# roysubhankar/dwt-domain-adaptation

Measured on NVIDIA H100. Metric: ResNet-50-DWT images/sec fwd+bwd, higher is better.
Workload: dtype f32

## Files before the change

dwt-domain-adaptation_b200/dwt_b200/csrc/norm_cl.cu:

```cuda
#include <stdlib.h>

#include <type_traits>

#include <cuda_bf16.h>

#include "dwt_common.cuh"
#include "norm_launch.h"
#include "small_algebra.cuh"

namespace dwt {
namespace {

constexpr int kT = 256;

__device__ __forceinline__ void pdl_wait() { asm volatile("griddepcontrol.wait;" ::: "memory"); }
__device__ __forceinline__ void pdl_launch_dependents() { asm volatile("griddepcontrol.launch_dependents;" ::: "memory"); }

template <int GS> struct ClShape {
  static constexpr int NSUB = 4 / GS;
  static constexpr int NM = GS * (GS + 1) / 2;
  static constexpr int FWD1 = GS + NM;
  static constexpr int BWD1 = GS * GS + GS;
  static constexpr int FWD = NSUB * FWD1;
  static constexpr int BWD = NSUB * BWD1;
};

struct ClThread {
  int C4, CW, LS, rpi, col, rsub, q;
  bool active;
  __device__ __forceinline__ ClThread(const Geom& gm) {
    C4 = gm.C >> 2;
    CW = gm.cw;
    LS = gm.ls;
    rpi = kT / LS;
    col = threadIdx.x % LS;
    rsub = threadIdx.x / LS;
    q = blockIdx.y * CW + col;
    active = col < CW && rsub < rpi && q < C4;
  }
};

template <int UNROLL, bool DESC, class F>
__device__ __forceinline__ void sweep_rows(const ClThread& t, unsigned rows, F&& body) {
  const unsigned krows = (unsigned)t.rpi * UNROLL, nch = (rows + krows - 1) / krows;
  for (unsigned i = blockIdx.x; i < nch; i += gridDim.x) body((DESC ? nch - 1 - i : i) * krows + t.rsub);
}
#define CL_FOR_DOMAINS(d, gm, DESC) \
  for (int di_ = blockIdx.z, d = (DESC) ? (gm).D - 1 - di_ : di_; di_ < (gm).D; di_ += gridDim.z, d = (DESC) ? (gm).D - 1 - di_ : di_)

template <class T> constexpr bool kBf16 = !std::is_same<T, float>::value;
template <class T>
__device__ __forceinline__ float as_stored(float v) {
  if constexpr (kBf16<T>) return __bfloat162float(__float2bfloat16_rn(v));
  else return v;
}

template <int NACC>
__device__ __forceinline__ void column_reduce(const ClThread& t, float (&acc)[NACC], float* sRed) {
  if (t.rpi == 1) return;
  if (t.rsub < t.rpi) {
#pragma unroll
    for (int i = 0; i < NACC; ++i) sRed[i * kT + threadIdx.x] = acc[i];
  }
  __syncthreads();
  if (t.rsub == 0) {
#pragma unroll
    for (int i = 0; i < NACC; ++i) {
      float s = acc[i];
      for (int r = 1; r < t.rpi; ++r) s += sRed[i * kT + r * t.LS + t.col];
      acc[i] = s;
    }
  }
}

template <class T, int GS>
__global__ void __launch_bounds__(kT, 3) cl_stats_kernel(const T* __restrict__ x, const Geom gm,
                                                         float* __restrict__ partial, float* __restrict__ shift) {
  using S = ClShape<GS>;
  constexpr int UNROLL = 8;
  __shared__ float sRed[kT * S::FWD];
  const ClThread t(gm);
  const unsigned rows = (unsigned)gm.N * gm.HW;
  pdl_launch_dependents();
  CL_FOR_DOMAINS(d, gm, true) {
    const T* xd = x + (size_t)d * rows * gm.C + 4 * t.q;
    float K[4] = {0.f, 0.f, 0.f, 0.f};
    if (t.active) {
      const unsigned np = rows < 8 ? rows : 8;
      for (unsigned r = 0; r < np; ++r) {
        const float4 v = ld4(xd + (size_t)r * gm.C);
        K[0] += v.x; K[1] += v.y; K[2] += v.z; K[3] += v.w;
      }
#pragma unroll
      for (int c = 0; c < 4; ++c) K[c] /= (float)np;
      if (rows > 8) {
        float s1[4] = {0.f, 0.f, 0.f, 0.f}, s2[4] = {0.f, 0.f, 0.f, 0.f};
        const size_t mid = (size_t)gm.HW / 2 + (size_t)sqrtf((float)gm.HW) / 2;
        for (unsigned k = 0; k < 8; ++k) {
          const float4 v = ld4(xd + ((2 * (size_t)k + 1) * rows / 16 + mid) % rows * gm.C);
          const float e[4] = {v.x - K[0], v.y - K[1], v.z - K[2], v.w - K[3]};
#pragma unroll
          for (int c = 0; c < 4; ++c) { s1[c] += e[c]; s2[c] = fmaf(e[c], e[c], s2[c]); }
        }
#pragma unroll
        for (int c = 0; c < 4; ++c) {
          const float dk = s1[c] * 0.125f;
          if (401.f * dk * dk > 400.f * (s2[c] * 0.125f)) K[c] += dk;
        }
      }
      if (blockIdx.x == 0 && t.rsub == 0) *reinterpret_cast<float4*>(shift + (size_t)d * gm.C + 4 * t.q) = make_float4(K[0], K[1], K[2], K[3]);
    }
    float acc[S::FWD];
#pragma unroll
    for (int i = 0; i < S::FWD; ++i) acc[i] = 0.f;
    if (t.active) sweep_rows<UNROLL, true>(t, rows, [&](unsigned r) {
      float4 v[UNROLL];
#pragma unroll
      for (int u = 0; u < UNROLL; ++u) {
        const unsigned rr = r + u * t.rpi;
        v[u] = rr < rows ? ld4(xd + (size_t)rr * gm.C) : make_float4(K[0], K[1], K[2], K[3]);
      }
#pragma unroll
      for (int u = 0; u < UNROLL; ++u) {
        const float e[4] = {v[u].x - K[0], v[u].y - K[1], v[u].z - K[2], v[u].w - K[3]};
#pragma unroll
        for (int s = 0; s < S::NSUB; ++s) {
#pragma unroll
          for (int c = 0; c < GS; ++c) {
            acc[s * S::FWD1 + c] += e[s * GS + c];
#pragma unroll
            for (int j = 0; j <= c; ++j)
              acc[s * S::FWD1 + GS + c * (c + 1) / 2 + j] = fmaf(e[s * GS + c], e[s * GS + j], acc[s * S::FWD1 + GS + c * (c + 1) / 2 + j]);
          }
        }
      }
    });
    column_reduce<S::FWD>(t, acc, sRed);
    if (t.rsub == 0 && t.active) {
      float* dst = partial + (((size_t)d * gridDim.x + blockIdx.x) * t.C4 + t.q) * S::FWD;
#pragma unroll
      for (int i = 0; i < S::FWD; ++i) dst[i] = acc[i];
    }
    if (gridDim.z == 1) __syncthreads();
  }
}

template <int GS, int PER>
__device__ __forceinline__ int acc_index(int g, int a) {
  constexpr int NSUB = 4 / GS;
  return (g / NSUB) * (NSUB * PER) + (g % NSUB) * PER + a;
}

constexpr int kFinQ = 2;

template <int NACC>
__device__ __forceinline__ void column_row_sum(const float* __restrict__ col, int nrows, int W, float (&a)[NACC]) {
  static_assert(NACC % 2 == 0, "accumulators are read as float2");
#pragma unroll
  for (int i = 0; i < NACC; ++i) a[i] = 0.f;
#pragma unroll 4
  for (int r = threadIdx.x; r < nrows; r += 32) {
    const float2* p = reinterpret_cast<const float2*>(col + (size_t)r * W);
#pragma unroll
    for (int i = 0; i < NACC / 2; ++i) {
      const float2 v = __ldcg(p + i);
      a[2 * i] += v.x; a[2 * i + 1] += v.y;
    }
  }
#pragma unroll
  for (int o = 1; o < 32; o <<= 1)
#pragma unroll
    for (int i = 0; i < NACC; ++i) a[i] += __shfl_xor_sync(0xffffffffu, a[i], o);
}

template <int NSUB, int PER>
__device__ __forceinline__ void take_group(const float (&a)[NSUB * PER], int s, float (&v)[PER]) {
#pragma unroll
  for (int i = 0; i < PER; ++i) {
    v[i] = a[i];
#pragma unroll
    for (int k = 1; k < NSUB; ++k)
      if (s == k) v[i] = a[k * PER + i];
  }
}

template <int GS>
__device__ __forceinline__ void cl_fwd_finalize_site(const float* __restrict__ partial, int nrows, const float* __restrict__ shift,
                                                     const Geom& gm, const FwdFin& fin) {
  using SH = ClShape<GS>;
  constexpr int NST = GS + GS * GS;
  __shared__ float sStat[DWT_MAX_DOMAINS][kFinQ][SH::NSUB][NST + 1];
  __shared__ unsigned char sBad[DWT_MAX_DOMAINS][kFinQ][SH::NSUB];
  const int s = threadIdx.x, ql = threadIdx.y, d = threadIdx.z, q = blockIdx.x * blockDim.y + ql;
  const int W = (gm.C >> 2) * SH::FWD;
  const float invM = 1.f / gm.M;
  const bool colok = q < (gm.C >> 2);
  const bool lead = colok && s < SH::NSUB;
  const int g = q * SH::NSUB + (lead ? s : 0);
  const bool direct = gm.D == 1 || fin.aliased == 0;
  const int dbuf = direct ? d : 0;
  const bool upd = fin.update_running && lead && (direct || (fin.aliased == 1 && d == 0));
  float rc_old[GS * GS], rm_old[GS];
  if (upd) {
#pragma unroll
    for (int e = 0; e < GS * GS; ++e) rc_old[e] = fin.rcov[dbuf][(size_t)g * GS * GS + e];
#pragma unroll
    for (int e = 0; e < GS; ++e) rm_old[e] = fin.rmean[dbuf][g * GS + e];
  }
  pdl_launch_dependents();
  pdl_wait();
  float a[SH::FWD];
  if (colok) column_row_sum<SH::FWD>(partial + (size_t)d * nrows * W + (size_t)q * SH::FWD, nrows, W, a);
  if (lead) {
    float v[SH::FWD1];
    take_group<SH::NSUB, SH::FWD1>(a, s, v);
    float mean[GS], cov[GS][GS];
#pragma unroll
    for (int i = 0; i < GS; ++i) mean[i] = shift[(size_t)d * gm.C + g * GS + i] + v[i] * invM;
#pragma unroll
    for (int i = 0; i < GS; ++i)
#pragma unroll
      for (int j = 0; j <= i; ++j) {
        const float c = v[GS + i * (i + 1) / 2 + j] * invM - (v[i] * invM) * (v[j] * invM);
        cov[i][j] = c; cov[j][i] = c;
      }
    const bool bad = factor_thread<GS>(gm, fin, d, g, mean, cov, false);
    if (fin.update_running) {
      if (direct) {
        if (!bad) {
          const float m = fin.momentum, kk = 1.f - fin.momentum;
#pragma unroll
          for (int i = 0; i < GS; ++i) {
            fin.rmean[d][g * GS + i] = m * mean[i] + kk * rm_old[i];
#pragma unroll
            for (int j = 0; j < GS; ++j)
              fin.rcov[d][(size_t)g * GS * GS + i * GS + j] = m * (cov[i][j] * fin.unbias) + kk * rc_old[i * GS + j];
          }
        }
      } else {
        sBad[d][ql][s] = bad ? 1 : 0;
#pragma unroll
        for (int i = 0; i < GS; ++i) {
          sStat[d][ql][s][i] = mean[i];
#pragma unroll
          for (int j = 0; j < GS; ++j) sStat[d][ql][s][GS + i * GS + j] = cov[i][j];
        }
      }
    }
  }
  if (!fin.update_running || direct) return;
  __syncthreads();
  if (!(lead && d == 0)) return;
  if (fin.aliased == 1) {
    const float m = fin.momentum, kk = 1.f - fin.momentum;
    float* rc = fin.rcov[0] + (size_t)g * GS * GS;
    float* rm = fin.rmean[0] + g * GS;
    for (int dd = 0; dd < gm.D; ++dd) {
      if (sBad[dd][ql][s]) continue;
#pragma unroll
      for (int e = 0; e < GS * GS; ++e) rc_old[e] = m * (sStat[dd][ql][s][GS + e] * fin.unbias) + kk * rc_old[e];
#pragma unroll
      for (int e = 0; e < GS; ++e) rm_old[e] = m * sStat[dd][ql][s][e] + kk * rm_old[e];
    }
#pragma unroll
    for (int e = 0; e < GS * GS; ++e) rc[e] = rc_old[e];
#pragma unroll
    for (int e = 0; e < GS; ++e) rm[e] = rm_old[e];
  } else {
    for (int dd = 0; dd < gm.D; ++dd)
      if (!sBad[dd][ql][s]) ema_direct<GS>(gm, fin, dd, g, &sStat[dd][ql][s][0], &sStat[dd][ql][s][GS]);
  }
}

template <int GS>
__global__ void __launch_bounds__(32 * kFinQ * DWT_MAX_DOMAINS) cl_fwd_finalize_kernel(const float* __restrict__ partial, size_t pstride, int nrows,
                                                                                      const float* __restrict__ shift, size_t sstride, const Geom gm,
                                                                                      const __grid_constant__ FwdFin fin, const __grid_constant__ FwdFin fin2) {
  const bool second = blockIdx.y != 0;
  cl_fwd_finalize_site<GS>(partial + (second ? pstride : 0), nrows, shift + (second ? sstride : 0), gm, second ? fin2 : fin);
}

template <class T, int GS, int EPI, bool DS>
__global__ void __launch_bounds__(kT, 3) cl_apply_kernel(const T* __restrict__ x, T* __restrict__ y, const Geom gm,
                                                         const float* __restrict__ save_mean, const float* __restrict__ save_w,
                                                         const float* __restrict__ gamma, const float* __restrict__ beta,
                                                         const T* __restrict__ res, uint8_t* __restrict__ mask,
                                                         const float* __restrict__ save_mean_d, const float* __restrict__ save_w_d,
                                                         const float* __restrict__ gamma_d, const float* __restrict__ beta_d) {
  using S = ClShape<GS>;
  constexpr bool RES = (EPI & DWT_EPI_RESIDUAL) != 0;
  static_assert(!DS || RES, "the two-site tail is a residual epilogue");
  constexpr int UNROLL = DS ? 2 : (RES ? 4 : 8);
  const ClThread t(gm);
  if (!t.active) return;
  const unsigned rows = (unsigned)gm.N * gm.HW;
  pdl_wait();
  CL_FOR_DOMAINS(d, gm, false) {
    float Wp[S::NSUB][S::NM], bp[S::NSUB][GS], Wd[DS ? S::NSUB : 1][S::NM], bd[DS ? S::NSUB : 1][GS];
#pragma unroll
    for (int s = 0; s < S::NSUB; ++s) {
      const int g = t.q * S::NSUB + s;
      load_forward_map<GS, EPI>(save_w + ((size_t)d * gm.G + g) * GS * GS, save_mean + (size_t)d * gm.C + g * GS,
                                gamma + g * GS, beta + g * GS, Wp[s], bp[s]);
      if constexpr (DS)
        load_forward_map<GS, DWT_EPI_AFFINE>(save_w_d + ((size_t)d * gm.G + g) * GS * GS, save_mean_d + (size_t)d * gm.C + g * GS,
                                             gamma_d + g * GS, beta_d + g * GS, Wd[s], bd[s]);
    }
    const size_t base = (size_t)d * rows * gm.C + 4 * t.q;
    const T* xd = x + base;
    const T* rd = res + base;
    T* yd = y + base;
    uint8_t* md = mask + (size_t)d * rows * t.C4 + t.q;
    sweep_rows<UNROLL, false>(t, rows, [&](unsigned r) {
      float4 v[UNROLL], rs[UNROLL];
#pragma unroll
      for (int u = 0; u < UNROLL; ++u) {
        const unsigned rr = r + u * t.rpi;
        if (rr < rows) {
          v[u] = ld4(xd + rr * (unsigned)gm.C);
          if constexpr (RES) rs[u] = ld4(rd + rr * (unsigned)gm.C);
        }
      }
#pragma unroll
      for (int u = 0; u < UNROLL; ++u) {
        const unsigned rr = r + u * t.rpi;
        if (rr < rows) {
          const float e[4] = {v[u].x, v[u].y, v[u].z, v[u].w};
          float o[4], ra[4] = {0.f, 0.f, 0.f, 0.f};
          if constexpr (RES) { ra[0] = rs[u].x; ra[1] = rs[u].y; ra[2] = rs[u].z; ra[3] = rs[u].w; }
          unsigned bits = 0;
#pragma unroll
          for (int s = 0; s < S::NSUB; ++s) {
            float xi[GS], oi[GS];
            if constexpr (DS) {
              float xdi[GS], odi[GS];
#pragma unroll
              for (int c = 0; c < GS; ++c) xdi[c] = ra[s * GS + c];
              apply_group<GS>(Wd[s], bd[s], xdi, odi);
#pragma unroll
              for (int c = 0; c < GS; ++c) ra[s * GS + c] = as_stored<T>(odi[c]);
            }
#pragma unroll
            for (int c = 0; c < GS; ++c) xi[c] = e[s * GS + c];
            apply_group<GS>(Wp[s], bp[s], xi, oi);
#pragma unroll
            for (int c = 0; c < GS; ++c) {
              const float z = RES ? oi[c] + ra[s * GS + c] : oi[c];
              if constexpr (RES) bits |= (z > 0.f ? 1u : 0u) << (s * GS + c);
              o[s * GS + c] = (EPI & DWT_EPI_RELU) ? fmaxf(z, 0.f) : z;
            }
          }
          st4(yd + rr * (unsigned)gm.C, make_float4(o[0], o[1], o[2], o[3]));
          if constexpr (RES) { if (mask != nullptr) md[rr * (unsigned)t.C4] = (uint8_t)bits; }
        }
      }
    });
  }
}

template <int GS>
__device__ __forceinline__ void bwd_accumulate(float* acc, const float (&dz)[GS], const float (&xi)[GS], const float* mu) {
#pragma unroll
  for (int i = 0; i < GS; ++i) {
    acc[GS * GS + i] += dz[i];
#pragma unroll
    for (int j = 0; j < GS; ++j) acc[i * GS + j] = fmaf(dz[i], xi[j] - mu[j], acc[i * GS + j]);
  }
}

template <class T, int GS, int EPI, bool D2, bool DS>
__global__ void __launch_bounds__(kT, 2) cl_bwd_reduce_kernel(const T* __restrict__ x, const T* __restrict__ dout, const T* __restrict__ dout2,
                                                              const Geom gm, const float* __restrict__ save_mean,
                                                              const float* __restrict__ save_w, const float* __restrict__ gamma,
                                                              const float* __restrict__ beta, const uint8_t* __restrict__ mask,
                                                              T* __restrict__ dzout, float* __restrict__ partial,
                                                              const T* __restrict__ xds, const float* __restrict__ save_mean_d,
                                                              size_t pstride) {
  using S = ClShape<GS>;
  constexpr int UNROLL = 4;
  constexpr bool MASK = (EPI & DWT_EPI_RESIDUAL) != 0;
  constexpr bool RELU = (EPI & DWT_EPI_RELU) != 0 && !MASK;
  static_assert(!DS || MASK, "the two-site tail is a residual epilogue");
  constexpr int NS = DS ? 2 : 1;
  __shared__ float sRed[kT * S::BWD];
  const ClThread t(gm);
  const unsigned rows = (unsigned)gm.N * gm.HW;
  pdl_launch_dependents();
  CL_FOR_DOMAINS(d, gm, true) {
    float Wp[S::NSUB][S::NM], bp[S::NSUB][GS], mu[NS][4];
    if (t.active) {
#pragma unroll
      for (int s = 0; s < S::NSUB; ++s) {
        const int g = t.q * S::NSUB + s;
        if constexpr (RELU)
          load_forward_map<GS, EPI>(save_w + ((size_t)d * gm.G + g) * GS * GS, save_mean + (size_t)d * gm.C + g * GS,
                                    gamma + g * GS, beta + g * GS, Wp[s], bp[s]);
      }
#pragma unroll
      for (int k = 0; k < NS; ++k) {
        const float4 m4 = ldg4((k ? save_mean_d : save_mean) + (size_t)d * gm.C + 4 * t.q);
        mu[k][0] = m4.x; mu[k][1] = m4.y; mu[k][2] = m4.z; mu[k][3] = m4.w;
      }
    }
    float acc[NS][S::BWD];
#pragma unroll
    for (int k = 0; k < NS; ++k)
#pragma unroll
      for (int i = 0; i < S::BWD; ++i) acc[k][i] = 0.f;
    const size_t base = (size_t)d * rows * gm.C + 4 * t.q;
    const T* xp[NS];
    xp[0] = x + base;
    if constexpr (DS) xp[NS - 1] = xds + base;
    const T* gd = dout + base;
    const T* gd2 = D2 ? dout2 + base : nullptr;
    T* zd = MASK ? dzout + base : nullptr;
    const uint8_t* md = mask + (size_t)d * rows * t.C4 + t.q;
    constexpr int H = DS ? UNROLL / 2 : UNROLL;
    if (t.active) sweep_rows<UNROLL, true>(t, rows, [&](unsigned r0) {
#pragma unroll
     for (int h = 0; h < UNROLL; h += H) {
      const unsigned r = r0 + h * t.rpi;
      float4 v[NS][H], q[H], q2[D2 ? H : 1];
      unsigned mb[H];
#pragma unroll
      for (int u = 0; u < H; ++u) {
        const unsigned rr = r + u * t.rpi;
        if (rr < rows) {
#pragma unroll
          for (int k = 0; k < NS; ++k) v[k][u] = ld4(xp[k] + (size_t)rr * gm.C);
          q[u] = ld4(gd + (size_t)rr * gm.C);
          if constexpr (MASK) mb[u] = __ldg(md + (size_t)rr * t.C4);
          if constexpr (D2) q2[u] = ld4(gd2 + (size_t)rr * gm.C);
        } else {
#pragma unroll
          for (int k = 0; k < NS; ++k) v[k][u] = make_float4(mu[k][0], mu[k][1], mu[k][2], mu[k][3]);
          q[u] = make_float4(0.f, 0.f, 0.f, 0.f);
          if constexpr (MASK) mb[u] = 0u;
          if constexpr (D2) q2[u] = make_float4(0.f, 0.f, 0.f, 0.f);
        }
      }
      if constexpr (D2) {
#pragma unroll
        for (int u = 0; u < H; ++u) {
          q[u].x = as_stored<T>(q[u].x + q2[u].x); q[u].y = as_stored<T>(q[u].y + q2[u].y);
          q[u].z = as_stored<T>(q[u].z + q2[u].z); q[u].w = as_stored<T>(q[u].w + q2[u].w);
        }
      }
#pragma unroll
      for (int u = 0; u < H; ++u) {
        const float ge[4] = {q[u].x, q[u].y, q[u].z, q[u].w};
        const float e[4] = {v[0][u].x, v[0][u].y, v[0][u].z, v[0][u].w};
        const float ed[4] = {v[NS - 1][u].x, v[NS - 1][u].y, v[NS - 1][u].z, v[NS - 1][u].w};
        float zm[4];
#pragma unroll
        for (int s = 0; s < S::NSUB; ++s) {
          float xi[GS], dz[GS];
#pragma unroll
          for (int c = 0; c < GS; ++c) { xi[c] = e[s * GS + c]; dz[c] = ge[s * GS + c]; }
          if constexpr (RELU) {
            float oi[GS];
            apply_group<GS>(Wp[s], bp[s], xi, oi);
#pragma unroll
            for (int c = 0; c < GS; ++c) dz[c] = oi[c] > 0.f ? dz[c] : 0.f;
          }
          if constexpr (MASK) {
#pragma unroll
            for (int c = 0; c < GS; ++c) { dz[c] = ((mb[u] >> (s * GS + c)) & 1u) ? dz[c] : 0.f; zm[s * GS + c] = dz[c]; }
          }
          bwd_accumulate<GS>(acc[0] + s * S::BWD1, dz, xi, &mu[0][s * GS]);
          if constexpr (DS) {
#pragma unroll
            for (int c = 0; c < GS; ++c) xi[c] = ed[s * GS + c];
            bwd_accumulate<GS>(acc[NS - 1] + s * S::BWD1, dz, xi, &mu[NS - 1][s * GS]);
          }
        }
        if constexpr (MASK) {
          const unsigned rr = r + u * t.rpi;
          if (rr < rows) st4(zd + (size_t)rr * gm.C, make_float4(zm[0], zm[1], zm[2], zm[3]));
        }
      }
     }
    });
#pragma unroll
    for (int k = 0; k < NS; ++k) {
      if (k) __syncthreads();
      column_reduce<S::BWD>(t, acc[k], sRed);
      if (t.rsub == 0 && t.active) {
        float* dst = partial + k * pstride + (((size_t)d * gridDim.x + blockIdx.x) * t.C4 + t.q) * S::BWD;
#pragma unroll
        for (int i = 0; i < S::BWD; ++i) dst[i] = acc[k][i];
      }
    }
    if (gridDim.z == 1) __syncthreads();
  }
}

template <int GS>
__device__ __forceinline__ void cl_bwd_finalize_site(const float* __restrict__ partial, int nrows, const Geom& gm, const BwdFin& fin) {
  using SH = ClShape<GS>;
  const int s = threadIdx.x, d = threadIdx.z, q = blockIdx.x * blockDim.y + threadIdx.y;
  const int W = (gm.C >> 2) * SH::BWD;
  const bool colok = q < (gm.C >> 2);
  pdl_launch_dependents();
  pdl_wait();
  float a[SH::BWD];
  if (colok) column_row_sum<SH::BWD>(partial + (size_t)d * nrows * W + (size_t)q * SH::BWD, nrows, W, a);
  if (colok && s < SH::NSUB) {
    float v[SH::BWD1], R[GS][GS], sdz[GS];
    take_group<SH::NSUB, SH::BWD1>(a, s, v);
#pragma unroll
    for (int i = 0; i < SH::BWD1; ++i) {
      if (i < GS * GS) R[i / GS][i % GS] = v[i]; else sdz[i - GS * GS] = v[i];
    }
    bwd_finalize_thread<GS>(gm, fin, d, q * SH::NSUB + s, R, sdz, false);
  }
  if (!((fin.epi & DWT_EPI_AFFINE) && fin.dgamma != nullptr)) return;
  __syncthreads();
  if (colok && d == 0 && s < 4) {
    const int ch = 4 * q + s;
    float sg = 0.f, sb = 0.f;
    for (int dd = 0; dd < gm.D; ++dd) {
      sg += fin.dgb_part[((size_t)dd * 2 + 0) * gm.C + ch];
      sb += fin.dgb_part[((size_t)dd * 2 + 1) * gm.C + ch];
    }
    fin.dgamma[ch] = sg;
    fin.dbeta[ch] = sb;
  }
}

template <int GS>
__global__ void __launch_bounds__(32 * kFinQ * DWT_MAX_DOMAINS) cl_bwd_finalize_kernel(const float* __restrict__ partial, size_t pstride, int nrows,
                                                                                      const Geom gm, const __grid_constant__ BwdFin fin,
                                                                                      const __grid_constant__ BwdFin fin2) {
  const bool second = blockIdx.y != 0;
  cl_bwd_finalize_site<GS>(partial + (second ? pstride : 0), nrows, gm, second ? fin2 : fin);
}

template <int GS>
struct BwdCoef {
  float A1[GS * (GS + 1) / 2], Bm[GS * (GS + 1) / 2], cv[GS];
  __device__ __forceinline__ void load(const float* cf) {
#pragma unroll
    for (int i = 0; i < GS; ++i) {
      cv[i] = __ldg(cf + 2 * GS * GS + i);
#pragma unroll
      for (int j = 0; j <= i; ++j) {
        A1[i * (i + 1) / 2 + j] = __ldg(cf + j * GS + i);
        Bm[i * (i + 1) / 2 + j] = __ldg(cf + GS * GS + i * GS + j);
      }
    }
  }
  __device__ __forceinline__ void apply(const float (&dz)[GS], const float (&xi)[GS], float* o) const {
#pragma unroll
    for (int i = 0; i < GS; ++i) {
      float a = cv[i];
#pragma unroll
      for (int j = i; j < GS; ++j) a = fmaf(A1[j * (j + 1) / 2 + i], dz[j], a);
#pragma unroll
      for (int j = 0; j < GS; ++j) {
        const int hi = i > j ? i : j, lo = i > j ? j : i;
        a = fmaf(Bm[hi * (hi + 1) / 2 + lo], xi[j], a);
      }
      o[i] = a;
    }
  }
};

template <class T, int GS, int EPI, bool D2, bool DS>
__global__ void __launch_bounds__(kT, 2) cl_bwd_apply_kernel(const T* __restrict__ x, const T* __restrict__ dout, const T* __restrict__ dout2,
                                                             T* __restrict__ dx, const Geom gm, const float* __restrict__ coef,
                                                             const float* __restrict__ save_mean, const float* __restrict__ save_w,
                                                             const float* __restrict__ gamma, const float* __restrict__ beta,
                                                             const T* __restrict__ xds, T* __restrict__ dxds,
                                                             const float* __restrict__ coef_d) {
  using S = ClShape<GS>;
  constexpr int UNROLL = 4;
  constexpr bool RELU = (EPI & DWT_EPI_RELU) != 0;
  static_assert((EPI & DWT_EPI_RESIDUAL) == 0, "the residual tail's apply runs with EPI = AFFINE on dz");
  static_assert(!DS || (!D2 && !RELU), "the two-site tail's apply reads dz");
  constexpr int NS = DS ? 2 : 1;
  const ClThread t(gm);
  if (!t.active) return;
  const unsigned rows = (unsigned)gm.N * gm.HW;
  pdl_wait();
  CL_FOR_DOMAINS(d, gm, false) {
    float Wp[S::NSUB][S::NM], bp[S::NSUB][GS];
    BwdCoef<GS> cf[NS][S::NSUB];
#pragma unroll
    for (int s = 0; s < S::NSUB; ++s) {
      const int g = t.q * S::NSUB + s;
      if constexpr (RELU)
        load_forward_map<GS, EPI>(save_w + ((size_t)d * gm.G + g) * GS * GS, save_mean + (size_t)d * gm.C + g * GS,
                                  gamma + g * GS, beta + g * GS, Wp[s], bp[s]);
#pragma unroll
      for (int k = 0; k < NS; ++k) cf[k][s].load((k ? coef_d : coef) + ((size_t)d * gm.G + g) * coef_stride(GS));
    }
    const size_t base = (size_t)d * rows * gm.C + 4 * t.q;
    const T* xp[NS];
    T* op[NS];
    xp[0] = x + base; op[0] = dx + base;
    if constexpr (DS) { xp[NS - 1] = xds + base; op[NS - 1] = dxds + base; }
    const T* gd = dout + base;
    const T* gd2 = D2 ? dout2 + base : nullptr;
    sweep_rows<UNROLL, false>(t, rows, [&](unsigned r) {
      float4 v[NS][UNROLL], q[UNROLL], q2[D2 ? UNROLL : 1];
#pragma unroll
      for (int u = 0; u < UNROLL; ++u) {
        const unsigned rr = r + u * t.rpi;
        if (rr < rows) {
#pragma unroll
          for (int k = 0; k < NS; ++k) v[k][u] = ld4(xp[k] + (size_t)rr * gm.C);
          q[u] = ld4(gd + (size_t)rr * gm.C);
          if constexpr (D2) q2[u] = ld4(gd2 + (size_t)rr * gm.C);
        }
      }
      if constexpr (D2) {
#pragma unroll
        for (int u = 0; u < UNROLL; ++u)
          if (r + u * t.rpi < rows) {
            q[u].x = as_stored<T>(q[u].x + q2[u].x); q[u].y = as_stored<T>(q[u].y + q2[u].y);
            q[u].z = as_stored<T>(q[u].z + q2[u].z); q[u].w = as_stored<T>(q[u].w + q2[u].w);
          }
      }
#pragma unroll
      for (int u = 0; u < UNROLL; ++u) {
        const unsigned rr = r + u * t.rpi;
        if (rr < rows) {
          const float ge[4] = {q[u].x, q[u].y, q[u].z, q[u].w};
#pragma unroll
          for (int k = 0; k < NS; ++k) {
            const float e[4] = {v[k][u].x, v[k][u].y, v[k][u].z, v[k][u].w};
            float o[4];
#pragma unroll
            for (int s = 0; s < S::NSUB; ++s) {
              float xi[GS], dz[GS];
#pragma unroll
              for (int c = 0; c < GS; ++c) { xi[c] = e[s * GS + c]; dz[c] = ge[s * GS + c]; }
              if constexpr (RELU) {
                float oi[GS];
                apply_group<GS>(Wp[s], bp[s], xi, oi);
#pragma unroll
                for (int c = 0; c < GS; ++c) dz[c] = oi[c] > 0.f ? dz[c] : 0.f;
              }
              cf[k][s].apply(dz, xi, o + s * GS);
            }
            st4(op[k] + (size_t)rr * gm.C, make_float4(o[0], o[1], o[2], o[3]));
          }
        }
      }
    });
  }
}

#define CL_GS(GS_, ...)                                  \
  switch (GS_) {                                         \
    case 1: { constexpr int kGS = 1; __VA_ARGS__; break; } \
    case 2: { constexpr int kGS = 2; __VA_ARGS__; break; } \
    case 4: { constexpr int kGS = 4; __VA_ARGS__; break; } \
    default: break;                                      \
  }
#define CL_EPI(E_, ...)                                                   \
  if ((E_) == 3) { constexpr int kEPI = 3; __VA_ARGS__; }                 \
  else if ((E_) == 1) { constexpr int kEPI = 1; __VA_ARGS__; }            \
  else { constexpr int kEPI = 0; __VA_ARGS__; }
#define CL_EPI_BWD(E_, ...)                                               \
  if ((E_) == 7) { constexpr int kEPI = 7; __VA_ARGS__; }                 \
  else CL_EPI(E_, __VA_ARGS__)
#define CL_D2(P_, ...)                                                    \
  if (P_) { constexpr bool kD2 = true; __VA_ARGS__; }                     \
  else { constexpr bool kD2 = false; __VA_ARGS__; }

inline bool use_pdl() {
  static const bool on = [] { const char* v = getenv("DWT_PDL"); return v != nullptr && v[0] == '1'; }();
  return on;
}

template <class... KArgs, class... Args>
inline void launch_k(void (*kernel)(KArgs...), dim3 grid, dim3 block, cudaStream_t st, bool pdl, Args... args) {
  cudaLaunchConfig_t cfg = {};
  cfg.gridDim = grid; cfg.blockDim = block; cfg.dynamicSmemBytes = 0; cfg.stream = st;
  cudaLaunchAttribute attr[1];
  attr[0].id = cudaLaunchAttributeProgrammaticStreamSerialization;
  attr[0].val.programmaticStreamSerializationAllowed = 1;
  cfg.attrs = attr; cfg.numAttrs = pdl ? 1 : 0;
  cudaLaunchKernelEx(&cfg, kernel, KArgs(args)...);
}

}

bool cl_supports(int C, int GS) {
  if (!(GS == 1 || GS == 2 || GS == 4) || C % 4 != 0) return false;
  const int c4 = C / 4;
  return c4 >= 1 && c4 <= 16384;
}

int cl_lane(int C, int CW) {
  if (C / 4 < 8) return CW;
  if (CW <= 32) {
    int l = 8;
    while (l < CW) l <<= 1;
    return l;
  }
  return (CW + 31) / 32 * 32;
}

namespace {
double cl_busy(int C4, int n) {
  const int cw = (C4 + n - 1) / n, last = C4 - (n - 1) * cw;
  if (cw < 8 || last <= 0) return -1.0;
  const int ls = cl_lane(4 * C4, cw);
  for (int v : {cw, last})
    if (ls <= 32 ? v < 8 : (v % 32 != 0 && v % 32 < 8)) return -1.0;
  return (double)C4 * (kT / ls) / ((double)n * kT);
}
}

int cl_slabs(int C) {
  const int C4 = C / 4;
  if ((C4 & (C4 - 1)) == 0) return C4 <= kT ? 1 : C4 / kT;
  if (C4 < 8) return 1;
  thread_local int memo_c = 0, memo_s = 0;
  if (memo_c == C) return memo_s;
  const int lo = (C4 + kT - 1) / kT, hi = C4 / 8;
  double top = 0.0;
  for (int n = lo; n <= hi; ++n) top = fmax(top, cl_busy(C4, n));
  int best = lo;
  for (int n = lo; n <= hi; ++n)
    if (cl_busy(C4, n) >= 0.0 && 64.0 * cl_busy(C4, n) >= 64.0 * top - 1.0) { best = n; break; }
  memo_c = C;
  memo_s = best;
  return best;
}

namespace {
inline dim3 cl_grid(const Geom& gm, int nctas, int gz) { return dim3(nctas, cl_slabs(gm.C), gz); }
inline Geom cl_geom(const Geom& gm) {
  Geom g = gm;
  const int C4 = gm.C / 4, slabs = cl_slabs(gm.C);
  g.cw = (C4 + slabs - 1) / slabs;
  g.ls = cl_lane(gm.C, g.cw);
  return g;
}
}
int cl_fwd_width(int C, int GS) { return (C / 4) * (4 / GS) * (GS + GS * (GS + 1) / 2); }
int cl_bwd_width(int C, int GS) { return (C / 4) * (4 / GS) * (GS * GS + GS); }


#define CL_T(BF16_, ...)                                                  \
  if (BF16_) { using TT = __nv_bfloat16; __VA_ARGS__; }                   \
  else { using TT = float; __VA_ARGS__; }
#define CL_IN(P_) static_cast<const TT*>(P_)
#define CL_OUT(P_) static_cast<TT*>(P_)

void cl_stats(const void* x, bool bf16, const Geom& gm, int nctas, int gz, float* partial, float* shift, cudaStream_t st) {
  CL_T(bf16, CL_GS(gm.GS, (cl_stats_kernel<TT, kGS><<<cl_grid(gm, nctas, gz), kT, 0, st>>>(CL_IN(x), cl_geom(gm), partial, shift))));
}
inline dim3 fin_block(const Geom& gm) { const int c4 = gm.C / 4; return dim3(32, c4 < kFinQ ? c4 : kFinQ, gm.D); }
inline unsigned fin_blocks(const Geom& gm, const dim3& b) { return (unsigned)((gm.C / 4 + b.y - 1) / b.y); }
void cl_fwd_finalize(const float* partial, int nrows, const float* shift, const Geom& gm, const FwdFin& fin, cudaStream_t st,
                     const FwdFin* fin2, size_t pstride, size_t sstride) {
  const dim3 b = fin_block(gm), g(fin_blocks(gm, b), fin2 ? 2 : 1);
  CL_GS(gm.GS, (launch_k(cl_fwd_finalize_kernel<kGS>, g, b, st, use_pdl(), partial, pstride, nrows, shift, sstride, gm, fin, fin2 ? *fin2 : fin)));
}
void cl_apply(const void* x, void* y, bool bf16, const Geom& gm, int nctas, int gz, int epi, const float* mean, const float* w,
              const float* gamma, const float* beta, const void* residual, uint8_t* mask, cudaStream_t st) {
  const float* nul = nullptr;
  CL_T(bf16, {
    const TT* tnul = nullptr;
    if (epi == 7) {
      CL_GS(gm.GS, (launch_k(cl_apply_kernel<TT, kGS, 7, false>, cl_grid(gm, nctas, gz), dim3(kT), st, use_pdl(), CL_IN(x), CL_OUT(y), cl_geom(gm), mean, w,
                             gamma, beta, CL_IN(residual), mask, nul, nul, nul, nul)));
    } else {
      CL_GS(gm.GS, CL_EPI(epi, (launch_k(cl_apply_kernel<TT, kGS, kEPI, false>, cl_grid(gm, nctas, gz), dim3(kT), st, use_pdl(), CL_IN(x), CL_OUT(y),
                                         cl_geom(gm), mean, w, gamma, beta, tnul, (uint8_t*)nullptr, nul, nul, nul, nul))));
    }
  });
}
void cl_tail2_apply(const void* x, const void* xd, void* y, bool bf16, const Geom& gm, int nctas, int gz, const float* mean, const float* w,
                    const float* gamma, const float* beta, const float* mean_d, const float* w_d, const float* gamma_d,
                    const float* beta_d, uint8_t* mask, cudaStream_t st) {
  CL_T(bf16, CL_GS(gm.GS, (launch_k(cl_apply_kernel<TT, kGS, 7, true>, cl_grid(gm, nctas, gz), dim3(kT), st, use_pdl(), CL_IN(x), CL_OUT(y), cl_geom(gm), mean,
                                    w, gamma, beta, CL_IN(xd), mask, mean_d, w_d, gamma_d, beta_d))));
}
void cl_bwd_reduce(const void* x, const void* dout, const void* dout2, bool bf16, const Geom& gm, int nctas, int gz, int epi, const float* mean,
                   const float* w, const float* gamma, const float* beta, const uint8_t* mask, void* dz, float* partial, cudaStream_t st) {
  const float* nul = nullptr;
  CL_T(bf16, {
    const TT* tnul = nullptr;
    CL_GS(gm.GS, CL_D2(dout2, CL_EPI_BWD(epi, (cl_bwd_reduce_kernel<TT, kGS, kEPI, kD2, false><<<cl_grid(gm, nctas, gz), kT, 0, st>>>(
                                                  CL_IN(x), CL_IN(dout), CL_IN(dout2), cl_geom(gm), mean, w, gamma, beta, mask, CL_OUT(dz), partial, tnul,
                                                  nul, 0)))));
  });
}
void cl_tail2_bwd_reduce(const void* x, const void* xd, const void* dout, const void* dout2, bool bf16, const Geom& gm, int nctas, int gz,
                         const float* mean, const float* mean_d, const uint8_t* mask, void* dz, float* partial, size_t pstride,
                         cudaStream_t st) {
  const float* nul = nullptr;
  CL_T(bf16, CL_GS(gm.GS, CL_D2(dout2, (cl_bwd_reduce_kernel<TT, kGS, 7, kD2, true><<<cl_grid(gm, nctas, gz), kT, 0, st>>>(
                                           CL_IN(x), CL_IN(dout), CL_IN(dout2), cl_geom(gm), mean, nul, nul, nul, mask, CL_OUT(dz), partial, CL_IN(xd),
                                           mean_d, pstride)))));
}
void cl_bwd_finalize(const float* partial, int nrows, const Geom& gm, const BwdFin& fin, cudaStream_t st, const BwdFin* fin2, size_t pstride) {
  const dim3 b = fin_block(gm), g(fin_blocks(gm, b), fin2 ? 2 : 1);
  CL_GS(gm.GS, (launch_k(cl_bwd_finalize_kernel<kGS>, g, b, st, use_pdl(), partial, pstride, nrows, gm, fin, fin2 ? *fin2 : fin)));
}
void cl_bwd_apply(const void* x, const void* dout, const void* dout2, void* dx, bool bf16, const Geom& gm, int nctas, int gz, int epi,
                  const float* coef, const float* mean, const float* w, const float* gamma, const float* beta, cudaStream_t st) {
  const float* nul = nullptr;
  CL_T(bf16, {
    const TT* tnul = nullptr;
    CL_GS(gm.GS, CL_D2(dout2, CL_EPI(epi, (launch_k(cl_bwd_apply_kernel<TT, kGS, kEPI, kD2, false>, cl_grid(gm, nctas, gz), dim3(kT), st, use_pdl(),
                                                    CL_IN(x), CL_IN(dout), CL_IN(dout2), CL_OUT(dx), cl_geom(gm), coef, mean, w, gamma, beta, tnul,
                                                    (TT*)nullptr, nul)))));
  });
}
void cl_tail2_bwd_apply(const void* x, const void* xd, const void* dz, void* dx, void* dxd, bool bf16, const Geom& gm, int nctas, int gz,
                        const float* coef, const float* coef_d, cudaStream_t st) {
  const float* nul = nullptr;
  CL_T(bf16, {
    const TT* tnul = nullptr;
    CL_GS(gm.GS, (launch_k(cl_bwd_apply_kernel<TT, kGS, 1, false, true>, cl_grid(gm, nctas, gz), dim3(kT), st, use_pdl(), CL_IN(x), CL_IN(dz), tnul,
                           CL_OUT(dx), cl_geom(gm), coef, nul, nul, nul, nul, CL_IN(xd), CL_OUT(dxd), coef_d)));
  });
}

}
```

Before: 3420.

## Software-pipeline row loads across grid-stride chunks with a register ring

Adds a ring-buffered row sweep that prefetches the next chunk's rows while the current chunk is being accumulated. The change applies to both the channels-last stats kernel and the backward reduction kernel, hiding global-load latency across chunk boundaries. It also batches the pilot-shift sample loads so they issue together, and replaces a modulo with a conditional subtract. The cost is more live registers, which could lower occupancy or cause spills under the existing launch bounds.

```diff
diff --git a/dwt-domain-adaptation_b200/dwt_b200/csrc/norm_cl.cu b/dwt-domain-adaptation_b200/dwt_b200/csrc/norm_cl.cu
--- a/dwt-domain-adaptation_b200/dwt_b200/csrc/norm_cl.cu
+++ b/dwt-domain-adaptation_b200/dwt_b200/csrc/norm_cl.cu
@@ -44,6 +44,34 @@
 __device__ __forceinline__ void sweep_rows(const ClThread& t, unsigned rows, F&& body) {
   const unsigned krows = (unsigned)t.rpi * UNROLL, nch = (rows + krows - 1) / krows;
   for (unsigned i = blockIdx.x; i < nch; i += gridDim.x) body((DESC ? nch - 1 - i : i) * krows + t.rsub);
+}
+
+template <int UNROLL, int P, bool DESC, class Row, class Load, class Use>
+__device__ __forceinline__ void sweep_rows_ring(const ClThread& t, unsigned rows, Load&& load, Use&& use) {
+  static_assert(UNROLL % P == 0, "the ring advances whole chunks");
+  const unsigned krows = (unsigned)t.rpi * UNROLL, nch = (rows + krows - 1) / krows;
+  auto first = [&](unsigned i) { return (DESC ? nch - 1 - i : i) * krows + t.rsub; };
+  unsigned i = blockIdx.x;
+  if (i >= nch) return;
+  unsigned r = first(i);
+  Row ring[P];
+#pragma unroll
+  for (int u = 0; u < P; ++u) ring[u] = load(r + u * t.rpi);
+  for (;;) {
+    const unsigned in = i + gridDim.x;
+    const bool more = in < nch;
+    const unsigned rn = more ? first(in) : 0u;
+#pragma unroll
+    for (int u = 0; u < UNROLL; ++u) {
+      const Row cur = ring[u % P];
+      if (u + P < UNROLL) ring[u % P] = load(r + (u + P) * t.rpi);
+      else if (more) ring[u % P] = load(rn + (u + P - UNROLL) * t.rpi);
+      use(cur, r + u * t.rpi);
+    }
+    if (!more) return;
+    i = in;
+    r = rn;
+  }
 }
 #define CL_FOR_DOMAINS(d, gm, DESC) \
   for (int di_ = blockIdx.z, d = (DESC) ? (gm).D - 1 - di_ : di_; di_ < (gm).D; di_ += gridDim.z, d = (DESC) ? (gm).D - 1 - di_ : di_)
@@ -87,42 +115,45 @@
     float K[4] = {0.f, 0.f, 0.f, 0.f};
     if (t.active) {
       const unsigned np = rows < 8 ? rows : 8;
-      for (unsigned r = 0; r < np; ++r) {
-        const float4 v = ld4(xd + (size_t)r * gm.C);
-        K[0] += v.x; K[1] += v.y; K[2] += v.z; K[3] += v.w;
-      }
+      float4 rowv[8];
+#pragma unroll
+      for (int k = 0; k < 8; ++k) rowv[k] = k < np ? ld4(xd + (size_t)k * gm.C) : make_float4(0.f, 0.f, 0.f, 0.f);
+#pragma unroll
+      for (int k = 0; k < 8; ++k) { K[0] += rowv[k].x; K[1] += rowv[k].y; K[2] += rowv[k].z; K[3] += rowv[k].w; }
 #pragma unroll
       for (int c = 0; c < 4; ++c) K[c] /= (float)np;
-      if (rows > 8) {
-        float s1[4] = {0.f, 0.f, 0.f, 0.f}, s2[4] = {0.f, 0.f, 0.f, 0.f};
-        const size_t mid = (size_t)gm.HW / 2 + (size_t)sqrtf((float)gm.HW) / 2;
-        for (unsigned k = 0; k < 8; ++k) {
-          const float4 v = ld4(xd + ((2 * (size_t)k + 1) * rows / 16 + mid) % rows * gm.C);
-          const float e[4] = {v.x - K[0], v.y - K[1], v.z - K[2], v.w - K[3]};
-#pragma unroll
-          for (int c = 0; c < 4; ++c) { s1[c] += e[c]; s2[c] = fmaf(e[c], e[c], s2[c]); }
-        }
-#pragma unroll
-        for (int c = 0; c < 4; ++c) {
-          const float dk = s1[c] * 0.125f;
-          if (401.f * dk * dk > 400.f * (s2[c] * 0.125f)) K[c] += dk;
-        }
-      }
-      if (blockIdx.x == 0 && t.rsub == 0) *reinterpret_cast<float4*>(shift + (size_t)d * gm.C + 4 * t.q) = make_float4(K[0], K[1], K[2], K[3]);
-    }
+    }
+    if (t.active && rows > 8) {
+      float4 rowv[8];
+      const unsigned mid = (unsigned)gm.HW / 2 + (unsigned)sqrtf((float)gm.HW) / 2;
+#pragma unroll
+      for (int k = 0; k < 8; ++k) {
+        const unsigned s = (unsigned)((2 * (size_t)k + 1) * rows / 16) + mid;
+        rowv[k] = ld4(xd + (size_t)(s >= rows ? s - rows : s) * gm.C);
+      }
+      float s1[4] = {0.f, 0.f, 0.f, 0.f}, s2[4] = {0.f, 0.f, 0.f, 0.f};
+#pragma unroll
+      for (int k = 0; k < 8; ++k) {
+        const float4 v = rowv[k];
+        const float e[4] = {v.x - K[0], v.y - K[1], v.z - K[2], v.w - K[3]};
+#pragma unroll
+        for (int c = 0; c < 4; ++c) { s1[c] += e[c]; s2[c] = fmaf(e[c], e[c], s2[c]); }
+      }
+#pragma unroll
+      for (int c = 0; c < 4; ++c) {
+        const float dk = s1[c] * 0.125f;
+        if (401.f * dk * dk > 400.f * (s2[c] * 0.125f)) K[c] += dk;
+      }
+    }
+    if (t.active && blockIdx.x == 0 && t.rsub == 0)
+      *reinterpret_cast<float4*>(shift + (size_t)d * gm.C + 4 * t.q) = make_float4(K[0], K[1], K[2], K[3]);
     float acc[S::FWD];
 #pragma unroll
     for (int i = 0; i < S::FWD; ++i) acc[i] = 0.f;
-    if (t.active) sweep_rows<UNROLL, true>(t, rows, [&](unsigned r) {
-      float4 v[UNROLL];
-#pragma unroll
-      for (int u = 0; u < UNROLL; ++u) {
-        const unsigned rr = r + u * t.rpi;
-        v[u] = rr < rows ? ld4(xd + (size_t)rr * gm.C) : make_float4(K[0], K[1], K[2], K[3]);
-      }
-#pragma unroll
-      for (int u = 0; u < UNROLL; ++u) {
-        const float e[4] = {v[u].x - K[0], v[u].y - K[1], v[u].z - K[2], v[u].w - K[3]};
+    if (t.active) sweep_rows_ring<UNROLL, UNROLL, true, float4>(t, rows,
+      [&](unsigned rr) { return rr < rows ? ld4(xd + (size_t)rr * gm.C) : make_float4(K[0], K[1], K[2], K[3]); },
+      [&](const float4& v, unsigned) {
+        const float e[4] = {v.x - K[0], v.y - K[1], v.z - K[2], v.w - K[3]};
 #pragma unroll
         for (int s = 0; s < S::NSUB; ++s) {
 #pragma unroll
@@ -133,8 +164,7 @@
               acc[s * S::FWD1 + GS + c * (c + 1) / 2 + j] = fmaf(e[s * GS + c], e[s * GS + j], acc[s * S::FWD1 + GS + c * (c + 1) / 2 + j]);
           }
         }
-      }
-    });
+      });
     column_reduce<S::FWD>(t, acc, sRed);
     if (t.rsub == 0 && t.active) {
       float* dst = partial + (((size_t)d * gridDim.x + blockIdx.x) * t.C4 + t.q) * S::FWD;
@@ -415,42 +445,34 @@
     const T* gd2 = D2 ? dout2 + base : nullptr;
     T* zd = MASK ? dzout + base : nullptr;
     const uint8_t* md = mask + (size_t)d * rows * t.C4 + t.q;
-    constexpr int H = DS ? UNROLL / 2 : UNROLL;
-    if (t.active) sweep_rows<UNROLL, true>(t, rows, [&](unsigned r0) {
-#pragma unroll
-     for (int h = 0; h < UNROLL; h += H) {
-      const unsigned r = r0 + h * t.rpi;
-      float4 v[NS][H], q[H], q2[D2 ? H : 1];
-      unsigned mb[H];
-#pragma unroll
-      for (int u = 0; u < H; ++u) {
-        const unsigned rr = r + u * t.rpi;
+    struct Row { float4 v[NS], q, q2; unsigned mb; };
+    if (t.active) sweep_rows_ring<UNROLL, DS ? UNROLL / 2 : UNROLL, true, Row>(t, rows,
+      [&](unsigned rr) {
+        Row w;
         if (rr < rows) {
 #pragma unroll
-          for (int k = 0; k < NS; ++k) v[k][u] = ld4(xp[k] + (size_t)rr * gm.C);
-          q[u] = ld4(gd + (size_t)rr * gm.C);
-          if constexpr (MASK) mb[u] = __ldg(md + (size_t)rr * t.C4);
-          if constexpr (D2) q2[u] = ld4(gd2 + (size_t)rr * gm.C);
+          for (int k = 0; k < NS; ++k) w.v[k] = ld4(xp[k] + (size_t)rr * gm.C);
+          w.q = ld4(gd + (size_t)rr * gm.C);
+          if constexpr (MASK) w.mb = __ldg(md + (size_t)rr * t.C4);
+          if constexpr (D2) w.q2 = ld4(gd2 + (size_t)rr * gm.C);
         } else {
 #pragma unroll
-          for (int k = 0; k < NS; ++k) v[k][u] = make_float4(mu[k][0], mu[k][1], mu[k][2], mu[k][3]);
-          q[u] = make_float4(0.f, 0.f, 0.f, 0.f);
-          if constexpr (MASK) mb[u] = 0u;
-          if constexpr (D2) q2[u] = make_float4(0.f, 0.f, 0.f, 0.f);
-        }
-      }
-      if constexpr (D2) {
-#pragma unroll
-        for (int u = 0; u < H; ++u) {
-          q[u].x = as_stored<T>(q[u].x + q2[u].x); q[u].y = as_stored<T>(q[u].y + q2[u].y);
-          q[u].z = as_stored<T>(q[u].z + q2[u].z); q[u].w = as_stored<T>(q[u].w + q2[u].w);
-        }
-      }
-#pragma unroll
-      for (int u = 0; u < H; ++u) {
-        const float ge[4] = {q[u].x, q[u].y, q[u].z, q[u].w};
-        const float e[4] = {v[0][u].x, v[0][u].y, v[0][u].z, v[0][u].w};
-        const float ed[4] = {v[NS - 1][u].x, v[NS - 1][u].y, v[NS - 1][u].z, v[NS - 1][u].w};
+          for (int k = 0; k < NS; ++k) w.v[k] = make_float4(mu[k][0], mu[k][1], mu[k][2], mu[k][3]);
+          w.q = make_float4(0.f, 0.f, 0.f, 0.f);
+          if constexpr (MASK) w.mb = 0u;
+          if constexpr (D2) w.q2 = make_float4(0.f, 0.f, 0.f, 0.f);
+        }
+        return w;
+      },
+      [&](const Row& w, unsigned rr) {
+        float4 q = w.q;
+        if constexpr (D2) {
+          q.x = as_stored<T>(q.x + w.q2.x); q.y = as_stored<T>(q.y + w.q2.y);
+          q.z = as_stored<T>(q.z + w.q2.z); q.w = as_stored<T>(q.w + w.q2.w);
+        }
+        const float ge[4] = {q.x, q.y, q.z, q.w};
+        const float e[4] = {w.v[0].x, w.v[0].y, w.v[0].z, w.v[0].w};
+        const float ed[4] = {w.v[NS - 1].x, w.v[NS - 1].y, w.v[NS - 1].z, w.v[NS - 1].w};
         float zm[4];
 #pragma unroll
         for (int s = 0; s < S::NSUB; ++s) {
@@ -465,7 +487,7 @@
           }
           if constexpr (MASK) {
 #pragma unroll
-            for (int c = 0; c < GS; ++c) { dz[c] = ((mb[u] >> (s * GS + c)) & 1u) ? dz[c] : 0.f; zm[s * GS + c] = dz[c]; }
+            for (int c = 0; c < GS; ++c) { dz[c] = ((w.mb >> (s * GS + c)) & 1u) ? dz[c] : 0.f; zm[s * GS + c] = dz[c]; }
           }
           bwd_accumulate<GS>(acc[0] + s * S::BWD1, dz, xi, &mu[0][s * GS]);
           if constexpr (DS) {
@@ -475,12 +497,9 @@
           }
         }
         if constexpr (MASK) {
-          const unsigned rr = r + u * t.rpi;
           if (rr < rows) st4(zd + (size_t)rr * gm.C, make_float4(zm[0], zm[1], zm[2], zm[3]));
         }
-      }
-     }
-    });
+      });
 #pragma unroll
     for (int k = 0; k < NS; ++k) {
       if (k) __syncthreads();
```

Result: no change. 3420 (median of 6 runs) (-0.0%).
